# a-slide/Quade

Measured on AMD Instinct MI355X. Metric: read-pairs/sec demultiplexed (2x150 bp, dual 8 bp index), higher is better.
Workload: dtype u8

## Files before the change

include/quade_hip.h:

```cpp
#ifndef QUADE_HIP_H
#define QUADE_HIP_H

#include <stdint.h>

#ifdef __cplusplus
extern "C" {
#endif

#define QD_ABI_VERSION 6

#define QD_OK 0
#define QD_ERR_INVALID (-1)
#define QD_ERR_NO_DEVICE (-2)
#define QD_ERR_HIP (-3)
#define QD_ERR_STATE (-4)
#define QD_ERR_UNSUPPORTED (-5)
#define QD_ERR_BARCODE (-6)
#define QD_ERR_FORMAT (-7)

#define QD_CODE_UNDETERMINED 0xFFFFu
#define QD_MAX_WINDOW 64
#define QD_MAX_KEY 32
#define QD_MAX_SAMPLES 32767

// ... 327 lines not shown
int qd_dev_filter(qd_ctx* ctx, const uint8_t* text1, int64_t len1, const uint32_t* recs1, const uint8_t* text2, int64_t len2,
                  const uint32_t* recs2, int64_t n_pairs, const uint16_t* codes, uint8_t* reasons);
int qd_dev_cstats(qd_ctx* ctx, const uint8_t* text1, int64_t len1, const uint32_t* recs1, const uint8_t* text2, int64_t len2,
                  const uint32_t* recs2, int64_t n_pairs, const uint16_t* codes, const uint8_t* drop);
#define QD_DEV_GUARD_BYTE 0xEE
int qd_dev_pack_rows(int device_id, const qd_layout* layout, const uint8_t* const text[2], const int64_t text_len[2],
                     const uint32_t* const recs[2], int64_t n, int64_t short_cap, uint8_t* const seq_rows[2], uint8_t* const qual_rows[2],
                     uint8_t* const len_rows[2], uint32_t* short_idx, int64_t short_room, uint32_t* n_short);
int qd_dev_route_format(int device_id, const qd_plan* plan, int32_t n_samples, int32_t write_pass, int32_t write_fail, int32_t write_undet,
                        const uint8_t* const text[4], const int64_t text_len[4], const uint32_t* const recs[4], const uint16_t* codes,
                        const uint8_t* drop, int64_t n, int32_t shift, uint16_t* dest, uint32_t* len1, uint32_t* len2, uint32_t* perm,
                        uint16_t* sdest, uint32_t* g1, uint32_t* g2, uint32_t* first, uint32_t* g1_first, uint32_t* g2_first, int64_t* base1,
                        int64_t* base2, uint8_t* out, int64_t out_cap, int64_t* out_used);
int qd_dev_pack_members(int device_id, const uint8_t* slots, int64_t stride, const uint32_t* len, int64_t n, uint64_t* offsets, uint8_t* packed,
                        int64_t packed_cap);
int qd_get_plan(const qd_ctx* ctx, qd_plan* out);
int qd_context_device(const qd_ctx* ctx, int32_t* device_id);

#ifdef __cplusplus
}
#endif
#endif
```

quade_amd/csrc/quade_text.hip:

```cpp
#include <hip/hip_runtime.h>

#include "quade_text.h"
#include "text_rules.h"

namespace {

constexpr uint32_t TILE = QD_TEXT_TILE;
constexpr uint32_t LINE_BLOCK = 256;
static_assert(LINE_BLOCK * 64 == TILE, "a lane owns 64 bytes of its tile");

struct __attribute__((packed, aligned(1))) U4 {
    uint32_t x, y, z, w;
};

__device__ __forceinline__ uint32_t nl_bits4(uint32_t w) {
    const uint32_t x = w ^ 0x0A0A0A0Au;
    const uint32_t t = ~(((x & 0x7F7F7F7Fu) + 0x7F7F7F7Fu) | x | 0x7F7F7F7Fu);
    return (((t >> 7) * 0x00204081u) >> 21) & 0xFu;
}

__device__ __forceinline__ uint64_t nl_mask64(const uint8_t* text, uint32_t b, uint32_t len, bool virt) {
    if (b > len) return 0;
    uint64_t m = 0;
    if (b < len) {
        const uint4* p = reinterpret_cast<const uint4*>(text + b);
#pragma unroll
        for (int q = 0; q < 4; ++q) {
            const uint4 v = p[q];
            const uint64_t bits = (uint64_t)nl_bits4(v.x) | ((uint64_t)nl_bits4(v.y) << 4) | ((uint64_t)nl_bits4(v.z) << 8) |
                                  ((uint64_t)nl_bits4(v.w) << 12);
            m |= bits << (16 * q);
        }
        if (len - b < 64) m &= (1ull << (len - b)) - 1;
    }
    if (virt && len - b < 64) m |= 1ull << (len - b);
    return m;
}

__device__ __forceinline__ bool virtual_newline(const uint8_t* text, uint32_t len, int at_eof) {
    return at_eof && len > 0 && text[len - 1] != '\n';
}

__device__ __forceinline__ uint32_t wave_scan_incl(uint32_t v, uint32_t lane) {
#pragma unroll
    for (int d = 1; d < 64; d <<= 1) {
        const uint32_t y = __shfl_up(v, d, 64);
        if (lane >= (uint32_t)d) v += y;
// ... 12 lines not shown
    const uint32_t inc = wave_scan_incl(v, lane);
    if (lane == 63) lds[wave] = inc;
    __syncthreads();
    uint32_t before = 0, all = 0;
#pragma unroll
    for (int i = 0; i < NW; ++i) {
        const uint32_t s = lds[i];
        if ((uint32_t)i < wave) before += s;
        all += s;
    }
    __syncthreads();
    *total = all;
    return before + inc - v;
}

__global__ __launch_bounds__(LINE_BLOCK) void line_count(const uint8_t* text, uint32_t len, int at_eof, uint32_t* tile_counts) {
    __shared__ uint32_t part[LINE_BLOCK / 64];
    const bool virt = virtual_newline(text, len, at_eof);
    const uint32_t b = blockIdx.x * TILE + threadIdx.x * 64u;
    const uint32_t c = wave_sum((uint32_t)__popcll(nl_mask64(text, b, len, virt)));
    if ((threadIdx.x & 63u) == 0) part[threadIdx.x >> 6] = c;
    __syncthreads();
    if (threadIdx.x == 0) tile_counts[blockIdx.x] = part[0] + part[1] + part[2] + part[3];
}

__global__ __launch_bounds__(1024) void scan_single(const uint32_t* in, uint32_t n, uint32_t* out) {
    __shared__ uint32_t lds[16];
    __shared__ uint32_t carry;
    if (threadIdx.x == 0) carry = 0;
    __syncthreads();
    for (uint32_t base = 0; base < n; base += 1024) {
        const uint32_t i = base + threadIdx.x;
        const uint32_t v = i < n ? in[i] : 0u;
        uint32_t total;
        const uint32_t ex = block_scan_excl<16>(v, lds, &total);
        const uint32_t c = carry;
        if (i < n) out[i] = c + ex;
        __syncthreads();
        if (threadIdx.x == 0) carry = c + total;
        __syncthreads();
    }
    if (threadIdx.x == 0) out[n] = carry;
}

struct ScanMany {
    const uint32_t* in[4];
    uint32_t* out[4];
    uint32_t n[4];
};
__global__ __launch_bounds__(1024) void scan_single_many(const ScanMany a) {
    __shared__ uint32_t lds[16];
    __shared__ uint32_t carry;
    const uint32_t* in = a.in[blockIdx.x];
    uint32_t* out = a.out[blockIdx.x];
    const uint32_t n = a.n[blockIdx.x];
    if (threadIdx.x == 0) carry = 0;
    __syncthreads();
    for (uint32_t base = 0; base < n; base += 1024) {
        const uint32_t i = base + threadIdx.x;
        const uint32_t v = i < n ? in[i] : 0u;
        uint32_t total;
        const uint32_t ex = block_scan_excl<16>(v, lds, &total);
        const uint32_t c = carry;
        if (i < n) out[i] = c + ex;
        __syncthreads();
        if (threadIdx.x == 0) carry = c + total;
        __syncthreads();
    }
    if (threadIdx.x == 0) out[n] = carry;
}
struct DoneMany {
    const uint32_t* a[4];
    const uint32_t* lines[4];
    uint32_t n[4];
    uint32_t cap[4];
    qd_scan_result* r[4];
};
__global__ void lines_done_many(const DoneMany d) {
    const uint32_t w = threadIdx.x;
    const uint32_t n = d.a[w][d.n[w]];
    qd_scan_result* r = d.r[w];
    r->n_lines = n;
    r->n_records = n / 4;
    r->overflow = n > d.cap[w] ? 1u : 0u;
    r->n_short = 0;
}
__global__ void recs_done_many(const DoneMany d) {
    const uint32_t w = threadIdx.x;
    qd_scan_result* r = d.r[w];
    const uint32_t n_rec = r->overflow ? 0u : r->n_records;
    const uint32_t n_tiles = (n_rec + 1024u - 1) / 1024u;
    r->n_kept = n_tiles <= d.n[w] ? d.a[w][n_tiles] : 0u;
    r->tail_start = n_rec ? d.lines[w][4 * n_rec - 1] + 1 : 0u;
}

__global__ void lines_done(const uint32_t* tile_base, uint32_t n_tiles, uint32_t line_cap, qd_scan_result* r) {
    const uint32_t n = tile_base[n_tiles];
    r->n_lines = n;
    r->n_records = n / 4;
    r->overflow = n > line_cap ? 1u : 0u;
    r->n_short = 0;
}

__global__ __launch_bounds__(LINE_BLOCK) void line_write(const uint8_t* text, uint32_t len, int at_eof, const uint32_t* tile_base,
                                                         uint32_t* lines, uint32_t line_cap) {
    __shared__ uint32_t lds[LINE_BLOCK / 64];
    const bool virt = virtual_newline(text, len, at_eof);
    const uint32_t b = blockIdx.x * TILE + threadIdx.x * 64u;
    uint64_t m = nl_mask64(text, b, len, virt);
    uint32_t total;
    uint32_t at = tile_base[blockIdx.x] + block_scan_excl<LINE_BLOCK / 64>((uint32_t)__popcll(m), lds, &total);
    while (m) {
        if (at < line_cap) lines[at] = b + (uint32_t)__builtin_ctzll(m);
        ++at;
        m &= m - 1;
    }
}

constexpr uint32_t REC_TILE = 1024;

struct Lines4 {
    uint32_t head, e0, e1, e2, e3;
};
__device__ __forceinline__ Lines4 record_lines(const uint32_t* lines, uint32_t r) {
    const uint4 e = reinterpret_cast<const uint4*>(lines)[r];
    Lines4 l;
    l.head = r ? lines[4 * r - 1] + 1 : 0u;
    l.e0 = e.x;
    l.e1 = e.y;
    l.e2 = e.z;
    l.e3 = e.w;
    return l;
}
__device__ __forceinline__ bool record_kept(const uint8_t* text, const Lines4& l, uint32_t* seq_len) {
    const uint32_t seq = l.e0 + 1, qual = l.e2 + 1;
    const uint32_t seq_end = (l.e1 > seq && text[l.e1 - 1] == '\r') ? l.e1 - 1 : l.e1;
    const uint32_t qual_end = (l.e3 > qual && text[l.e3 - 1] == '\r') ? l.e3 - 1 : l.e3;
    *seq_len = seq_end - seq;
    return seq_end - seq == qual_end - qual;
}

__global__ __launch_bounds__(256) void rec_count(const uint8_t* text, const uint32_t* lines, const qd_scan_result* res, uint32_t need,
                                                 uint32_t* rec_tile, qd_scan_result* out) {
    __shared__ uint32_t part[4], parts[4];
    const uint32_t n_rec = res->overflow ? 0u : res->n_records;
    uint32_t kept = 0, shorts = 0;
#pragma unroll
    for (int i = 0; i < 4; ++i) {
        const uint32_t r = blockIdx.x * REC_TILE + threadIdx.x * 4u + (uint32_t)i;
        if (r < n_rec) {
            uint32_t sl;
            if (record_kept(text, record_lines(lines, r), &sl)) {
                ++kept;
                shorts += sl < need ? 1u : 0u;
            }
        }
    }
    kept = wave_sum(kept);
    shorts = wave_sum(shorts);
    if ((threadIdx.x & 63u) == 0) {
        part[threadIdx.x >> 6] = kept;
        parts[threadIdx.x >> 6] = shorts;
    }
    __syncthreads();
    if (threadIdx.x == 0) {
        rec_tile[blockIdx.x] = part[0] + part[1] + part[2] + part[3];
        const uint32_t s = parts[0] + parts[1] + parts[2] + parts[3];
        if (s) atomicAdd(&out->n_short, s);
    }
}

__global__ void recs_done(const uint32_t* rec_tile, uint32_t n_tiles_max, const uint32_t* lines, qd_scan_result* r) {
    const uint32_t n_rec = r->overflow ? 0u : r->n_records;
    const uint32_t n_tiles = (n_rec + REC_TILE - 1) / REC_TILE;
    r->n_kept = n_tiles <= n_tiles_max ? rec_tile[n_tiles] : 0u;
    r->tail_start = n_rec ? lines[4 * n_rec - 1] + 1 : 0u;
}

__device__ __forceinline__ void name_of_wide(const uint8_t* text, uint32_t head, uint32_t line_end, uint32_t* name_off, uint32_t* name_len) {
    uint32_t h = head + (line_end > head ? 1u : 0u);
    while (h < line_end && qd_is_blank(text[h])) ++h;
    uint32_t e = h;
    while (e < line_end) {
        uint64_t v;
        __builtin_memcpy(&v, text + e, 8);
        uint32_t k = 8;
#pragma unroll
        for (int i = 7; i >= 0; --i)
            if (qd_is_blank((uint8_t)(v >> (8 * i)))) k = (uint32_t)i;
        e += k;
        if (k < 8) break;
    }
    if (e > line_end) e = line_end;
    *name_off = h;
    *name_len = e - h;
}

__global__ __launch_bounds__(256) void rec_write(const uint8_t* text, const uint32_t* lines, const qd_scan_result* res, int want_names,
                                                 const uint32_t* rec_tile, qd_rec* recs) {
    __shared__ uint32_t lds[4];
    const uint32_t n_rec = res->overflow ? 0u : res->n_records;
    Lines4 l[4];
    uint32_t sl[4];
    bool keep[4];
    uint32_t kept = 0;
#pragma unroll
    for (int i = 0; i < 4; ++i) {
        const uint32_t r = blockIdx.x * REC_TILE + threadIdx.x * 4u + (uint32_t)i;
        keep[i] = false;
        if (r < n_rec) {
            l[i] = record_lines(lines, r);
            keep[i] = record_kept(text, l[i], &sl[i]);
        }
        kept += keep[i] ? 1u : 0u;
    }
    uint32_t total;
    uint32_t at = rec_tile[blockIdx.x] + block_scan_excl<4>(kept, lds, &total);
#pragma unroll
    for (int i = 0; i < 4; ++i) {
        if (!keep[i]) continue;
        qd_rec q;
        q.head = l[i].head;
        q.seq = l[i].e0 + 1;
        q.seq_len = sl[i];
        q.qual = l[i].e2 + 1;
        q.name_off = q.head;
        q.name_len = 0;
        if (want_names) name_of_wide(text, l[i].head, l[i].e0, &q.name_off, &q.name_len);
        recs[at++] = q;
    }
}

__global__ void carry_info(const qd_rec* r0, const qd_rec* r1, const qd_rec* r2, const qd_rec* r3, qd_scan_result* s0, qd_scan_result* s1,
                           qd_scan_result* s2, qd_scan_result* s3, int n_streams, uint32_t n0, uint32_t n1, uint32_t n2, uint32_t n3) {
    const qd_rec* recs[4] = {r0, r1, r2, r3};
    qd_scan_result* res[4] = {s0, s1, s2, s3};
    const uint32_t ns[4] = {n0, n1, n2, n3};
    const int k = (int)threadIdx.x;
    if (k < n_streams) res[k]->carry_start = ns[k] < res[k]->n_kept ? recs[k][ns[k]].head : res[k]->tail_start;
}

__global__ void grain_bounds(const uint32_t* lines, const qd_scan_result* res, const uint32_t* grain_start, uint32_t n_grains, qd_grain_index* out) {
    const uint32_t g = blockIdx.x * blockDim.x + threadIdx.x;
    if (g >= n_grains) return;
// ... 432 lines not shown
    const uint32_t i = blockIdx.x;
    const uint32_t L = len[i];
    const uint32_t b0 = blockIdx.y * COPY_PART;
    if (b0 >= L) return;
    const uint32_t b1 = min(b0 + COPY_PART, L);
    const uint8_t* s = slots + (int64_t)i * stride;
    uint8_t* d = packed + offsets[i];
    uint32_t b = b0 + threadIdx.x * 16u;
    for (; b + 16 <= b1; b += 256 * 16) *reinterpret_cast<U4*>(d + b) = *reinterpret_cast<const U4*>(s + b);
    if (b < b1)
        for (uint32_t q = b; q < b1; ++q) d[q] = s[q];
}

}

hipError_t qd_text_scan(const uint8_t* text, uint32_t len, int at_eof, int want_names, uint32_t need, const qd_scan_scratch& s,
                        qd_scan_result* result, hipStream_t st) {
    const uint32_t n_tiles = len / TILE + 1;
    hipLaunchKernelGGL(line_count, dim3(n_tiles), dim3(LINE_BLOCK), 0, st, text, len, at_eof, s.tile_counts);
    hipLaunchKernelGGL(scan_single, dim3(1), dim3(1024), 0, st, s.tile_counts, n_tiles, s.tile_base);
    hipLaunchKernelGGL(lines_done, dim3(1), dim3(1), 0, st, s.tile_base, n_tiles, s.line_cap, result);
    hipLaunchKernelGGL(line_write, dim3(n_tiles), dim3(LINE_BLOCK), 0, st, text, len, at_eof, s.tile_base, s.lines, s.line_cap);
    const uint32_t rec_cap = s.line_cap / 4;
    const uint32_t rec_tiles = (rec_cap + REC_TILE - 1) / REC_TILE;
    if (rec_tiles) {
        hipLaunchKernelGGL(rec_count, dim3(rec_tiles), dim3(256), 0, st, text, s.lines, result, need, s.rec_tile, result);
        hipLaunchKernelGGL(scan_single, dim3(1), dim3(1024), 0, st, s.rec_tile, rec_tiles, s.rec_tile);
        hipLaunchKernelGGL(recs_done, dim3(1), dim3(1), 0, st, s.rec_tile, rec_tiles, s.lines, result);
        hipLaunchKernelGGL(rec_write, dim3(rec_tiles), dim3(256), 0, st, text, s.lines, result, want_names, s.rec_tile, s.recs);
    } else {
        hipLaunchKernelGGL(recs_done, dim3(1), dim3(1), 0, st, s.rec_tile, 0u, s.lines, result);
    }
    return hipGetLastError();
}

hipError_t qd_text_scan_many(int n_windows, const qd_scan_job* jobs, hipStream_t st) {
    if (n_windows < 1 || n_windows > 4) return hipErrorInvalidValue;
    static_assert(REC_TILE == 1024, "recs_done_many");
    ScanMany sm{}, sr{};
    DoneMany dl{}, dr{};
    uint32_t n_tiles[4], rec_tiles[4];
    bool any_rec = false;
    for (int w = 0; w < n_windows; ++w) {
        const qd_scan_job& j = jobs[w];
        n_tiles[w] = j.len / TILE + 1;
        rec_tiles[w] = (j.s.line_cap / 4 + REC_TILE - 1) / REC_TILE;
        any_rec = any_rec || rec_tiles[w];
        sm.in[w] = j.s.tile_counts, sm.out[w] = j.s.tile_base, sm.n[w] = n_tiles[w];
        sr.in[w] = j.s.rec_tile, sr.out[w] = j.s.rec_tile, sr.n[w] = rec_tiles[w];
        dl.a[w] = j.s.tile_base, dl.n[w] = n_tiles[w], dl.cap[w] = j.s.line_cap, dl.r[w] = j.result;
        dr.a[w] = j.s.rec_tile, dr.lines[w] = j.s.lines, dr.n[w] = rec_tiles[w], dr.r[w] = j.result;
    }
    for (int w = 0; w < n_windows; ++w)
        hipLaunchKernelGGL(line_count, dim3(n_tiles[w]), dim3(LINE_BLOCK), 0, st, jobs[w].text, jobs[w].len, jobs[w].at_eof, jobs[w].s.tile_counts);
    hipLaunchKernelGGL(scan_single_many, dim3(n_windows), dim3(1024), 0, st, sm);
    hipLaunchKernelGGL(lines_done_many, dim3(1), dim3(n_windows), 0, st, dl);
    for (int w = 0; w < n_windows; ++w)
        hipLaunchKernelGGL(line_write, dim3(n_tiles[w]), dim3(LINE_BLOCK), 0, st, jobs[w].text, jobs[w].len, jobs[w].at_eof, jobs[w].s.tile_base, jobs[w].s.lines, jobs[w].s.line_cap);
    for (int w = 0; w < n_windows; ++w)
        if (rec_tiles[w])
            hipLaunchKernelGGL(rec_count, dim3(rec_tiles[w]), dim3(256), 0, st, jobs[w].text, jobs[w].s.lines, jobs[w].result, jobs[w].need, jobs[w].s.rec_tile, jobs[w].result);
    if (any_rec) hipLaunchKernelGGL(scan_single_many, dim3(n_windows), dim3(1024), 0, st, sr);
    hipLaunchKernelGGL(recs_done_many, dim3(1), dim3(n_windows), 0, st, dr);
    for (int w = 0; w < n_windows; ++w)
        if (rec_tiles[w])
            hipLaunchKernelGGL(rec_write, dim3(rec_tiles[w]), dim3(256), 0, st, jobs[w].text, jobs[w].s.lines, jobs[w].result, jobs[w].want_names, jobs[w].s.rec_tile, jobs[w].s.recs);
    return hipGetLastError();
}

hipError_t qd_text_grain_index(const uint8_t* text, const uint32_t* lines, uint32_t line_cap, const qd_scan_result* res, const uint32_t* grain_start,
                               uint32_t n_grains, int at_eof, qd_grain_index* out, hipStream_t st) {
    if (!n_grains) return hipSuccess;
    hipLaunchKernelGGL(grain_bounds, dim3((n_grains + 63) / 64), dim3(64), 0, st, lines, res, grain_start, n_grains, out);
    if (line_cap) hipLaunchKernelGGL(grain_index, dim3((line_cap + 255) / 256), dim3(256), 0, st, text, lines, res, grain_start, n_grains, at_eof, out);
    return hipGetLastError();
}

hipError_t qd_text_carry_info(const qd_rec* const recs[4], qd_scan_result* const results[4], int n_streams, const uint32_t n[4], hipStream_t st) {
    hipLaunchKernelGGL(carry_info, dim3(1), dim3(64), 0, st, recs[0], recs[1], recs[2], recs[3], results[0], results[1], results[2], results[3],
                       n_streams, n[0], n[1], n[2], n[3]);
    return hipGetLastError();
}
// ... 102 lines not shown
```

quade_amd/csrc/quade_text_api.cpp:

```cpp
#include <hip/hip_runtime.h>

#include <cstring>
#include <string>
#include <vector>

#include "../../include/quade_hip.h"
#include "quade_text.h"

namespace {
struct Dev {
    void* p = nullptr;
    ~Dev() {
        if (p) (void)hipFree(p);
    }
    hipError_t alloc(size_t n) { return hipMalloc(&p, n ? n : 16); }
    template <class T>
    T* as() { return static_cast<T*>(p); }
};
#define TCHK(call)                            \
    do {                                      \
        if ((call) != hipSuccess) return QD_ERR_HIP; \
    } while (0)
}

// ... 19 lines not shown
    sc.tile_counts = tc.as<uint32_t>();
    sc.tile_base = tb.as<uint32_t>();
    sc.lines = lines.as<uint32_t>();
    sc.line_cap = (uint32_t)line_cap;
    sc.rec_tile = rt.as<uint32_t>();
    sc.recs = recs.as<qd_rec>();
    TCHK(qd_text_scan(d_text.as<uint8_t>(), len, at_eof, want_names, (uint32_t)need, sc, res.as<qd_scan_result>(), nullptr));
    TCHK(hipDeviceSynchronize());
    qd_scan_result r;
    TCHK(hipMemcpy(&r, res.p, sizeof r, hipMemcpyDeviceToHost));
    memcpy(result_out, &r, sizeof r);
    if (r.overflow) return 0;
    const int64_t n = std::min<int64_t>(r.n_kept, recs_cap);
    if (n && recs_out) TCHK(hipMemcpy(recs_out, recs.p, (size_t)n * sizeof(qd_rec), hipMemcpyDeviceToHost));
    return r.n_kept;
}

int qd_dev_crc32(int device_id, const uint8_t* data, int64_t n, int64_t range_bytes, uint32_t* crc_out) {
    if ((!data && n) || n < 0 || range_bytes < 1 || range_bytes > 65536 || !crc_out) return QD_ERR_INVALID;
    TCHK(hipSetDevice(device_id));
    std::vector<qd_crc_range> ranges;
    for (int64_t a = 0; a < n; a += range_bytes) ranges.push_back(qd_crc_range{(uint64_t)a + 3, (uint32_t)std::min<int64_t>(range_bytes, n - a), 0});
    const uint32_t first[2] = {0, (uint32_t)ranges.size()};
    Dev d, dr, dc, df, out;
    TCHK(d.alloc((size_t)n + 16));
    TCHK(dr.alloc(ranges.size() * sizeof(qd_crc_range)));
    TCHK(dc.alloc(ranges.size() * 4));
    TCHK(df.alloc(8));
    TCHK(out.alloc(4));
    if (n) TCHK(hipMemcpy(d.as<uint8_t>() + 3, data, (size_t)n, hipMemcpyHostToDevice));
// ... 239 lines not shown
```

quade_amd/hip_backend.py:

```python
from __future__ import annotations

import ctypes as C
import os

import numpy as np

_HERE = os.path.dirname(os.path.abspath(__file__))
LIB_PATH = os.path.join(_HERE, "lib", "libquade_hip.so")

QD_OK = 0
QD_ERR_INVALID, QD_ERR_NO_DEVICE, QD_ERR_HIP, QD_ERR_STATE = -1, -2, -3, -4
QD_ERR_UNSUPPORTED, QD_ERR_BARCODE, QD_ERR_FORMAT = -5, -6, -7
QD_UNKNOWN_READ_ERROR = -(1 << 40)
CODE_UNDETERMINED = 0xFFFF


class QuadeHipError(RuntimeError):
    def __init__(self, code, text):
        RuntimeError.__init__(self, "libquade_hip error %d: %s" % (code, text))
        self.code = code


class qd_plan(C.Structure):
    _fields_ = [("dual", C.c_int32), ("min_qual", C.c_int32),
# ... 190 lines not shown
    ("qd_dev_crc32", C.c_int, [C.c_int, _P, C.c_int64, C.c_int64, C.POINTER(C.c_uint32)]),
    ("qd_pool_trim", C.c_int, []),
    ("qd_dev_gunzip", C.c_int, [C.c_int, _P, C.c_int64, _P, C.c_int64, C.POINTER(C.c_int64), C.c_int64, C.c_int64, C.c_int64, C.POINTER(C.c_int64)]),
    ("qd_dev_sort_by_dest", C.c_int, [C.c_int, _P, C.c_int64, C.c_int32, _P, _P, _P]),
    ("qd_dev_qstats", C.c_int, [_P, _P, C.c_int64, _P, _P, C.c_int64, _P, C.c_int64, _P]),
    ("qd_dev_clip", C.c_int, [_P, _P, C.c_int64, _P, _P, C.c_int64, _P, C.c_int64, _P, _P]),
    ("qd_dev_trim", C.c_int, [_P, _P, C.c_int64, _P, _P, C.c_int64, _P, C.c_int64, _P, _P]),
    ("qd_dev_pairtrim", C.c_int, [_P, _P, C.c_int64, _P, _P, C.c_int64, _P, C.c_int64, _P, _P]),
    ("qd_dev_filter", C.c_int, [_P, _P, C.c_int64, _P, _P, C.c_int64, _P, C.c_int64, _P, _P]),
    ("qd_dev_cstats", C.c_int, [_P, _P, C.c_int64, _P, _P, C.c_int64, _P, C.c_int64, _P, _P]),
    ("qd_dev_pack_rows", C.c_int, [C.c_int, C.POINTER(qd_layout), _P * 2, C.c_int64 * 2, _P * 2, C.c_int64, C.c_int64, _P * 2, _P * 2, _P * 2,
                                   _P, C.c_int64, C.POINTER(C.c_uint32)]),
    ("qd_dev_route_format", C.c_int, [C.c_int, C.POINTER(qd_plan), C.c_int32, C.c_int32, C.c_int32, C.c_int32, _P * 4, C.c_int64 * 4, _P * 4, _P, _P,
                                      C.c_int64, C.c_int32] + [_P] * 13 + [C.c_int64, C.POINTER(C.c_int64)]),
    ("qd_dev_pack_members", C.c_int, [C.c_int, _P, C.c_int64, _P, C.c_int64, _P, _P, C.c_int64]),
    ("qd_get_plan", C.c_int, [_P, C.POINTER(qd_plan)]),
    ("qd_context_device", C.c_int, [_P, C.POINTER(C.c_int32)]),
]

_lib = None


def load_library(path=None):
    global _lib
    if _lib is not None and path is None:
        return _lib
    default = path is None
    path = path or os.environ.get("QUADE_HIP_LIB") or LIB_PATH
    if not os.path.exists(path):
        raise ImportError(
# ... 854 lines not shown
def dev_pack_members(slots, stride, lens, packed_cap, device_id=0):
    lib = load_library()
    lens = np.ascontiguousarray(lens, dtype=np.uint32)
    slots = np.ascontiguousarray(slots, dtype=np.uint8)
    n = lens.size
    assert slots.size >= n * int(stride)
    offsets = np.zeros(n + 1, dtype=np.uint64)
    packed = np.zeros(max(int(packed_cap), 1), dtype=np.uint8)
    rc = lib.qd_dev_pack_members(int(device_id), _ptr(slots) if n else None, int(stride), _ptr(lens) if n else None, n, _ptr(offsets), _ptr(packed),
                                 int(packed_cap))
    if rc != QD_OK:
        raise QuadeHipError(rc, "qd_dev_pack_members: " + lib.qd_strerror(rc).decode())
    return offsets, packed[:int(packed_cap)]


class Pipe(object):

    def __init__(self, engine, batch_pairs=None):
        self.lib = load_library()
        self.engine = engine
        h = _P()
        r = self.lib.qd_pipe_create(engine._h, C.byref(h))
        if r != QD_OK:
            raise QuadeHipError(r, self.lib.qd_pipe_last_error(None).decode())
        self._h = h
        if batch_pairs:
            self.set_option("batch_pairs", batch_pairs)

    def set_option(self, name, value):
        r = self.lib.qd_pipe_set_option(self._h, name.encode(), int(value))
# ... 58 lines not shown
```

Baseline: 177.4 billion.

## Batch FASTQ scan kernels across windows and skip record compaction when none dropped

The line-count, line-write and record kernels now take all windows in one launch, with each block finding its window from a per-window first-block table. The separate scan and done kernels are merged, which cuts the number of kernel launches. Tiles also record whether they contain any carriage return, so the common CR-free case can skip the per-record CR check. A new fused rec_pass writes records directly and counts drops, so the count, scan and compacting write run only when some record was actually dropped. The cost is extra indirection per block, and a drop-count flag that every later kernel must read before it can exit early.

Measured after the change: 177.2 billion. Within noise of the previous version (-0.1%).

```diff
diff --git a/include/quade_hip.h b/include/quade_hip.h
--- a/include/quade_hip.h
+++ b/include/quade_hip.h
@@ -365,6 +365,10 @@
                         int64_t* base2, uint8_t* out, int64_t out_cap, int64_t* out_used);
 int qd_dev_pack_members(int device_id, const uint8_t* slots, int64_t stride, const uint32_t* len, int64_t n, uint64_t* offsets, uint8_t* packed,
                         int64_t packed_cap);
+int qd_dev_fastq_scan_many(int device_id, int32_t n_windows, const uint8_t* const text[4], const int64_t text_len[4], const int32_t at_eof[4],
+                           const int32_t want_names[4], const int32_t need[4], const int64_t line_cap[4], uint32_t* const lines_out[4],
+                           uint32_t* const recs_out[4], const int64_t recs_cap[4], uint32_t* result_out, int32_t* guards_changed,
+                           int32_t timed_runs, float* ms_out);
 int qd_get_plan(const qd_ctx* ctx, qd_plan* out);
 int qd_context_device(const qd_ctx* ctx, int32_t* device_id);
 
diff --git a/quade_amd/csrc/quade_text.hip b/quade_amd/csrc/quade_text.hip
--- a/quade_amd/csrc/quade_text.hip
+++ b/quade_amd/csrc/quade_text.hip
@@ -1,4 +1,6 @@
 #include <hip/hip_runtime.h>
+
+#include <algorithm>
 
 #include "quade_text.h"
 #include "text_rules.h"
@@ -18,19 +20,27 @@
     const uint32_t t = ~(((x & 0x7F7F7F7Fu) + 0x7F7F7F7Fu) | x | 0x7F7F7F7Fu);
     return (((t >> 7) * 0x00204081u) >> 21) & 0xFu;
 }
-
-__device__ __forceinline__ uint64_t nl_mask64(const uint8_t* text, uint32_t b, uint32_t len, bool virt) {
+__device__ __forceinline__ uint32_t cr_in4(uint32_t w) {
+    const uint32_t x = w ^ 0x0D0D0D0Du;
+    return (x - 0x01010101u) & ~x & 0x80808080u;
+}
+
+__device__ __forceinline__ uint64_t nl_mask64(const uint8_t* text, uint32_t b, uint32_t len, bool virt, uint32_t* cr = nullptr) {
+    if (cr) *cr = 0;
     if (b > len) return 0;
     uint64_t m = 0;
     if (b < len) {
         const uint4* p = reinterpret_cast<const uint4*>(text + b);
+        uint32_t any_cr = 0;
 #pragma unroll
         for (int q = 0; q < 4; ++q) {
             const uint4 v = p[q];
             const uint64_t bits = (uint64_t)nl_bits4(v.x) | ((uint64_t)nl_bits4(v.y) << 4) | ((uint64_t)nl_bits4(v.z) << 8) |
                                   ((uint64_t)nl_bits4(v.w) << 12);
             m |= bits << (16 * q);
-        }
+            any_cr |= cr_in4(v.x) | cr_in4(v.y) | cr_in4(v.z) | cr_in4(v.w);
+        }
+        if (cr) *cr = any_cr;
         if (len - b < 64) m &= (1ull << (len - b)) - 1;
     }
     if (virt && len - b < 64) m |= 1ull << (len - b);
@@ -73,102 +83,105 @@
     return before + inc - v;
 }
 
-__global__ __launch_bounds__(LINE_BLOCK) void line_count(const uint8_t* text, uint32_t len, int at_eof, uint32_t* tile_counts) {
-    __shared__ uint32_t part[LINE_BLOCK / 64];
-    const bool virt = virtual_newline(text, len, at_eof);
-    const uint32_t b = blockIdx.x * TILE + threadIdx.x * 64u;
-    const uint32_t c = wave_sum((uint32_t)__popcll(nl_mask64(text, b, len, virt)));
-    if ((threadIdx.x & 63u) == 0) part[threadIdx.x >> 6] = c;
-    __syncthreads();
-    if (threadIdx.x == 0) tile_counts[blockIdx.x] = part[0] + part[1] + part[2] + part[3];
-}
-
+__device__ __forceinline__ uint32_t scan_words(const uint32_t* in, uint32_t n, uint32_t* out, uint32_t* lds , uint32_t* carry,
+                                               uint32_t mask = 0xFFFFFFFFu, uint32_t* rest = nullptr) {
+    uint32_t others = 0;
+    if (threadIdx.x == 0) *carry = 0;
+    __syncthreads();
+    for (uint32_t base = 0; base < n; base += 1024) {
+        const uint32_t i = base + threadIdx.x;
+        const uint32_t word = i < n ? in[i] : 0u;
+        const uint32_t v = word & mask;
+        others |= word & ~mask;
+        uint32_t total;
+        const uint32_t ex = block_scan_excl<16>(v, lds, &total);
+        const uint32_t c = *carry;
+        if (i < n) out[i] = c + ex;
+        __syncthreads();
+        if (threadIdx.x == 0) *carry = c + total;
+        __syncthreads();
+    }
+    const uint32_t all = *carry;
+    if (threadIdx.x == 0) out[n] = all;
+    if (rest) *rest = others;
+    return all;
+}
 __global__ __launch_bounds__(1024) void scan_single(const uint32_t* in, uint32_t n, uint32_t* out) {
     __shared__ uint32_t lds[16];
     __shared__ uint32_t carry;
-    if (threadIdx.x == 0) carry = 0;
-    __syncthreads();
-    for (uint32_t base = 0; base < n; base += 1024) {
-        const uint32_t i = base + threadIdx.x;
-        const uint32_t v = i < n ? in[i] : 0u;
-        uint32_t total;
-        const uint32_t ex = block_scan_excl<16>(v, lds, &total);
-        const uint32_t c = carry;
-        if (i < n) out[i] = c + ex;
-        __syncthreads();
-        if (threadIdx.x == 0) carry = c + total;
-        __syncthreads();
-    }
-    if (threadIdx.x == 0) out[n] = carry;
-}
-
-struct ScanMany {
-    const uint32_t* in[4];
-    uint32_t* out[4];
-    uint32_t n[4];
+    scan_words(in, n, out, lds, &carry);
+}
+
+__device__ __forceinline__ uint32_t window_of(const uint32_t first[5], uint32_t block) {
+    return (block >= first[1] ? 1u : 0u) + (block >= first[2] ? 1u : 0u) + (block >= first[3] ? 1u : 0u);
+}
+
+struct LineJobs {
+    const uint8_t* text[4];
+    uint32_t len[4];
+    int at_eof[4];
+    uint32_t* tile_counts[4];
+    const uint32_t* tile_base[4];
+    uint32_t* lines[4];
+    uint32_t line_cap[4];
+    uint32_t first[5];
 };
-__global__ __launch_bounds__(1024) void scan_single_many(const ScanMany a) {
+
+constexpr uint32_t TILE_HAS_CR = 0x80000000u;
+__global__ __launch_bounds__(LINE_BLOCK) void line_count(const LineJobs j) {
+    __shared__ uint32_t part[LINE_BLOCK / 64];
+    const uint32_t w = window_of(j.first, blockIdx.x), tile = blockIdx.x - j.first[w];
+    const uint8_t* text = j.text[w];
+    const uint32_t len = j.len[w], lane = threadIdx.x & 63u, wave = threadIdx.x >> 6;
+    const bool virt = virtual_newline(text, len, j.at_eof[w]);
+    uint32_t cr;
+    uint32_t c = wave_sum((uint32_t)__popcll(nl_mask64(text, tile * TILE + threadIdx.x * 64u, len, virt, &cr)));
+    if (__any(cr != 0)) c |= TILE_HAS_CR;
+    if (lane == 0) part[wave] = c;
+    __syncthreads();
+    if (threadIdx.x == 0) {
+        const uint32_t cr_bit = (part[0] | part[1] | part[2] | part[3]) & TILE_HAS_CR;
+        j.tile_counts[w][tile] = (((part[0] & ~TILE_HAS_CR) + (part[1] & ~TILE_HAS_CR) + (part[2] & ~TILE_HAS_CR) + (part[3] & ~TILE_HAS_CR))) | cr_bit;
+    }
+}
+
+struct LineScan {
+    const uint32_t* tile_counts[4];
+    uint32_t* tile_base[4];
+    uint32_t n_tiles[4];
+    uint32_t line_cap[4];
+    uint32_t* dropped[4];
+    qd_scan_result* r[4];
+};
+__global__ __launch_bounds__(1024) void line_scan(const LineScan a) {
     __shared__ uint32_t lds[16];
     __shared__ uint32_t carry;
-    const uint32_t* in = a.in[blockIdx.x];
-    uint32_t* out = a.out[blockIdx.x];
-    const uint32_t n = a.n[blockIdx.x];
-    if (threadIdx.x == 0) carry = 0;
-    __syncthreads();
-    for (uint32_t base = 0; base < n; base += 1024) {
-        const uint32_t i = base + threadIdx.x;
-        const uint32_t v = i < n ? in[i] : 0u;
-        uint32_t total;
-        const uint32_t ex = block_scan_excl<16>(v, lds, &total);
-        const uint32_t c = carry;
-        if (i < n) out[i] = c + ex;
-        __syncthreads();
-        if (threadIdx.x == 0) carry = c + total;
-        __syncthreads();
-    }
-    if (threadIdx.x == 0) out[n] = carry;
-}
-struct DoneMany {
-    const uint32_t* a[4];
-    const uint32_t* lines[4];
-    uint32_t n[4];
-    uint32_t cap[4];
-    qd_scan_result* r[4];
-};
-__global__ void lines_done_many(const DoneMany d) {
-    const uint32_t w = threadIdx.x;
-    const uint32_t n = d.a[w][d.n[w]];
-    qd_scan_result* r = d.r[w];
-    r->n_lines = n;
-    r->n_records = n / 4;
-    r->overflow = n > d.cap[w] ? 1u : 0u;
-    r->n_short = 0;
-}
-__global__ void recs_done_many(const DoneMany d) {
-    const uint32_t w = threadIdx.x;
-    qd_scan_result* r = d.r[w];
-    const uint32_t n_rec = r->overflow ? 0u : r->n_records;
-    const uint32_t n_tiles = (n_rec + 1024u - 1) / 1024u;
-    r->n_kept = n_tiles <= d.n[w] ? d.a[w][n_tiles] : 0u;
-    r->tail_start = n_rec ? d.lines[w][4 * n_rec - 1] + 1 : 0u;
-}
-
-__global__ void lines_done(const uint32_t* tile_base, uint32_t n_tiles, uint32_t line_cap, qd_scan_result* r) {
-    const uint32_t n = tile_base[n_tiles];
-    r->n_lines = n;
-    r->n_records = n / 4;
-    r->overflow = n > line_cap ? 1u : 0u;
-    r->n_short = 0;
-}
-
-__global__ __launch_bounds__(LINE_BLOCK) void line_write(const uint8_t* text, uint32_t len, int at_eof, const uint32_t* tile_base,
-                                                         uint32_t* lines, uint32_t line_cap) {
+    const uint32_t w = blockIdx.x;
+    uint32_t cr;
+    const uint32_t n = scan_words(a.tile_counts[w], a.n_tiles[w], a.tile_base[w], lds, &carry, ~TILE_HAS_CR, &cr);
+    cr = (uint32_t)__syncthreads_or((int)(cr != 0));
+    if (threadIdx.x == 0) {
+        qd_scan_result* r = a.r[w];
+        r->n_lines = n;
+        r->n_records = n / 4;
+        r->overflow = n > a.line_cap[w] ? 1u : 0u;
+        r->n_short = 0;
+        a.dropped[w][0] = 0;
+        a.dropped[w][1] = cr;
+    }
+}
+
+__global__ __launch_bounds__(LINE_BLOCK) void line_write(const LineJobs j) {
     __shared__ uint32_t lds[LINE_BLOCK / 64];
-    const bool virt = virtual_newline(text, len, at_eof);
-    const uint32_t b = blockIdx.x * TILE + threadIdx.x * 64u;
+    const uint32_t w = window_of(j.first, blockIdx.x), tile = blockIdx.x - j.first[w];
+    const uint8_t* text = j.text[w];
+    const uint32_t len = j.len[w], line_cap = j.line_cap[w];
+    uint32_t* lines = j.lines[w];
+    const bool virt = virtual_newline(text, len, j.at_eof[w]);
+    const uint32_t b = tile * TILE + threadIdx.x * 64u;
     uint64_t m = nl_mask64(text, b, len, virt);
     uint32_t total;
-    uint32_t at = tile_base[blockIdx.x] + block_scan_excl<LINE_BLOCK / 64>((uint32_t)__popcll(m), lds, &total);
+    uint32_t at = j.tile_base[w][tile] + block_scan_excl<LINE_BLOCK / 64>((uint32_t)__popcll(m), lds, &total);
     while (m) {
         if (at < line_cap) lines[at] = b + (uint32_t)__builtin_ctzll(m);
         ++at;
@@ -191,49 +204,12 @@
     l.e3 = e.w;
     return l;
 }
-__device__ __forceinline__ bool record_kept(const uint8_t* text, const Lines4& l, uint32_t* seq_len) {
+__device__ __forceinline__ bool record_kept(const uint8_t* text, const Lines4& l, uint32_t* seq_len, bool has_cr = true) {
     const uint32_t seq = l.e0 + 1, qual = l.e2 + 1;
-    const uint32_t seq_end = (l.e1 > seq && text[l.e1 - 1] == '\r') ? l.e1 - 1 : l.e1;
-    const uint32_t qual_end = (l.e3 > qual && text[l.e3 - 1] == '\r') ? l.e3 - 1 : l.e3;
+    const uint32_t seq_end = (has_cr && l.e1 > seq && text[l.e1 - 1] == '\r') ? l.e1 - 1 : l.e1;
+    const uint32_t qual_end = (has_cr && l.e3 > qual && text[l.e3 - 1] == '\r') ? l.e3 - 1 : l.e3;
     *seq_len = seq_end - seq;
     return seq_end - seq == qual_end - qual;
-}
-
-__global__ __launch_bounds__(256) void rec_count(const uint8_t* text, const uint32_t* lines, const qd_scan_result* res, uint32_t need,
-                                                 uint32_t* rec_tile, qd_scan_result* out) {
-    __shared__ uint32_t part[4], parts[4];
-    const uint32_t n_rec = res->overflow ? 0u : res->n_records;
-    uint32_t kept = 0, shorts = 0;
-#pragma unroll
-    for (int i = 0; i < 4; ++i) {
-        const uint32_t r = blockIdx.x * REC_TILE + threadIdx.x * 4u + (uint32_t)i;
-        if (r < n_rec) {
-            uint32_t sl;
-            if (record_kept(text, record_lines(lines, r), &sl)) {
-                ++kept;
-                shorts += sl < need ? 1u : 0u;
-            }
-        }
-    }
-    kept = wave_sum(kept);
-    shorts = wave_sum(shorts);
-    if ((threadIdx.x & 63u) == 0) {
-        part[threadIdx.x >> 6] = kept;
-        parts[threadIdx.x >> 6] = shorts;
-    }
-    __syncthreads();
-    if (threadIdx.x == 0) {
-        rec_tile[blockIdx.x] = part[0] + part[1] + part[2] + part[3];
-        const uint32_t s = parts[0] + parts[1] + parts[2] + parts[3];
-        if (s) atomicAdd(&out->n_short, s);
-    }
-}
-
-__global__ void recs_done(const uint32_t* rec_tile, uint32_t n_tiles_max, const uint32_t* lines, qd_scan_result* r) {
-    const uint32_t n_rec = r->overflow ? 0u : r->n_records;
-    const uint32_t n_tiles = (n_rec + REC_TILE - 1) / REC_TILE;
-    r->n_kept = n_tiles <= n_tiles_max ? rec_tile[n_tiles] : 0u;
-    r->tail_start = n_rec ? lines[4 * n_rec - 1] + 1 : 0u;
 }
 
 __device__ __forceinline__ void name_of_wide(const uint8_t* text, uint32_t head, uint32_t line_end, uint32_t* name_off, uint32_t* name_len) {
@@ -254,18 +230,132 @@
     *name_off = h;
     *name_len = e - h;
 }
-
-__global__ __launch_bounds__(256) void rec_write(const uint8_t* text, const uint32_t* lines, const qd_scan_result* res, int want_names,
-                                                 const uint32_t* rec_tile, qd_rec* recs) {
+__device__ __forceinline__ qd_rec record_of(const uint8_t* text, const Lines4& l, uint32_t seq_len, int want_names) {
+    qd_rec q;
+    q.head = l.head;
+    q.seq = l.e0 + 1;
+    q.seq_len = seq_len;
+    q.qual = l.e2 + 1;
+    q.name_off = q.head;
+    q.name_len = 0;
+    if (want_names) name_of_wide(text, l.head, l.e0, &q.name_off, &q.name_len);
+    return q;
+}
+
+struct RecJobs {
+    const uint8_t* text[4];
+    const uint32_t* lines[4];
+    qd_scan_result* res[4];
+    uint32_t need[4];
+    int want_names[4];
+    uint32_t* rec_tile[4];
+    qd_rec* recs[4];
+    uint32_t* dropped[4];
+    uint32_t first[5];
+};
+
+__global__ __launch_bounds__(256) void rec_pass(const RecJobs j) {
+    __shared__ uint32_t part[4], parts[4];
+    const uint32_t w = window_of(j.first, blockIdx.x), tile = blockIdx.x - j.first[w];
+    qd_scan_result* res = j.res[w];
+    const uint32_t n_rec = res->overflow ? 0u : res->n_records;
+    if (tile * REC_TILE >= n_rec) return;
+    const uint8_t* text = j.text[w];
+    const uint32_t* lines = j.lines[w];
+    const uint32_t need = j.need[w];
+    const int want_names = j.want_names[w];
+    qd_rec* recs = j.recs[w];
+    const bool has_cr = j.dropped[w][1] != 0;
+    uint32_t drops = 0, shorts = 0;
+#pragma unroll
+    for (uint32_t i = 0; i < 4; ++i) {
+        const uint32_t r = tile * REC_TILE + i * 256u + threadIdx.x;
+        if (r >= n_rec) continue;
+        const Lines4 l = record_lines(lines, r);
+        uint32_t sl;
+        if (record_kept(text, l, &sl, has_cr)) {
+            shorts += sl < need ? 1u : 0u;
+            recs[r] = record_of(text, l, sl, want_names);
+        } else {
+            ++drops;
+        }
+    }
+    drops = wave_sum(drops);
+    shorts = wave_sum(shorts);
+    if ((threadIdx.x & 63u) == 0) {
+        part[threadIdx.x >> 6] = drops;
+        parts[threadIdx.x >> 6] = shorts;
+    }
+    __syncthreads();
+    if (threadIdx.x == 0) {
+        const uint32_t d = part[0] + part[1] + part[2] + part[3], s = parts[0] + parts[1] + parts[2] + parts[3];
+        if (d) atomicAdd(j.dropped[w], d);
+        if (s) atomicAdd(&res->n_short, s);
+    }
+}
+
+__global__ __launch_bounds__(256) void rec_count(const RecJobs j) {
+    __shared__ uint32_t part[4];
+    const uint32_t w = window_of(j.first, blockIdx.x), tile = blockIdx.x - j.first[w];
+    if (*j.dropped[w] == 0) return;
+    const qd_scan_result* res = j.res[w];
+    const uint32_t n_rec = res->overflow ? 0u : res->n_records;
+    if (tile * REC_TILE >= n_rec) return;
+    const uint8_t* text = j.text[w];
+    const uint32_t* lines = j.lines[w];
+    uint32_t kept = 0;
+#pragma unroll
+    for (int i = 0; i < 4; ++i) {
+        const uint32_t r = tile * REC_TILE + threadIdx.x * 4u + (uint32_t)i;
+        if (r < n_rec) {
+            uint32_t sl;
+            kept += record_kept(text, record_lines(lines, r), &sl) ? 1u : 0u;
+        }
+    }
+    kept = wave_sum(kept);
+    if ((threadIdx.x & 63u) == 0) part[threadIdx.x >> 6] = kept;
+    __syncthreads();
+    if (threadIdx.x == 0) j.rec_tile[w][tile] = part[0] + part[1] + part[2] + part[3];
+}
+
+struct RecScan {
+    uint32_t* rec_tile[4];
+    const uint32_t* lines[4];
+    const uint32_t* dropped[4];
+    qd_scan_result* r[4];
+};
+__global__ __launch_bounds__(1024) void rec_scan(const RecScan a) {
+    __shared__ uint32_t lds[16];
+    __shared__ uint32_t carry;
+    const uint32_t w = blockIdx.x;
+    qd_scan_result* r = a.r[w];
+    const uint32_t n_rec = r->overflow ? 0u : r->n_records;
+    uint32_t n_kept = n_rec;
+    if (*a.dropped[w] != 0) n_kept = scan_words(a.rec_tile[w], (n_rec + REC_TILE - 1) / REC_TILE, a.rec_tile[w], lds, &carry);
+    if (threadIdx.x == 0) {
+        r->n_kept = n_kept;
+        r->tail_start = n_rec ? a.lines[w][4 * n_rec - 1] + 1 : 0u;
+    }
+}
+
+__global__ __launch_bounds__(256) void rec_write(const RecJobs j) {
     __shared__ uint32_t lds[4];
+    const uint32_t w = window_of(j.first, blockIdx.x), tile = blockIdx.x - j.first[w];
+    if (*j.dropped[w] == 0) return;
+    const qd_scan_result* res = j.res[w];
     const uint32_t n_rec = res->overflow ? 0u : res->n_records;
+    if (tile * REC_TILE >= n_rec) return;
+    const uint8_t* text = j.text[w];
+    const uint32_t* lines = j.lines[w];
+    const int want_names = j.want_names[w];
+    qd_rec* recs = j.recs[w];
     Lines4 l[4];
     uint32_t sl[4];
     bool keep[4];
     uint32_t kept = 0;
 #pragma unroll
     for (int i = 0; i < 4; ++i) {
-        const uint32_t r = blockIdx.x * REC_TILE + threadIdx.x * 4u + (uint32_t)i;
+        const uint32_t r = tile * REC_TILE + threadIdx.x * 4u + (uint32_t)i;
         keep[i] = false;
         if (r < n_rec) {
             l[i] = record_lines(lines, r);
@@ -274,19 +364,11 @@
         kept += keep[i] ? 1u : 0u;
     }
     uint32_t total;
-    uint32_t at = rec_tile[blockIdx.x] + block_scan_excl<4>(kept, lds, &total);
+    uint32_t at = j.rec_tile[w][tile] + block_scan_excl<4>(kept, lds, &total);
 #pragma unroll
     for (int i = 0; i < 4; ++i) {
         if (!keep[i]) continue;
-        qd_rec q;
-        q.head = l[i].head;
-        q.seq = l[i].e0 + 1;
-        q.seq_len = sl[i];
-        q.qual = l[i].e2 + 1;
-        q.name_off = q.head;
-        q.name_len = 0;
-        if (want_names) name_of_wide(text, l[i].head, l[i].e0, &q.name_off, &q.name_len);
-        recs[at++] = q;
+        recs[at++] = record_of(text, l[i], sl[i], want_names);
     }
 }
 
@@ -749,58 +831,45 @@
 
 }
 
+hipError_t qd_text_scan_many(int n_windows, const qd_scan_job* jobs, hipStream_t st) {
+    if (n_windows < 1 || n_windows > 4) return hipErrorInvalidValue;
+    LineJobs lj{};
+    LineScan ls{};
+    RecJobs rj{};
+    RecScan rs{};
+    uint32_t line_tiles = 0, rec_tiles = 0;
+    for (int w = 0; w < n_windows; ++w) {
+        const qd_scan_job& j = jobs[w];
+        const uint32_t n_tiles = j.len / TILE + 1;
+        const uint32_t rec_cap = (uint32_t)std::min<uint64_t>(j.s.line_cap, (uint64_t)j.len + 1) / 4;
+        uint32_t* dropped = j.s.tile_counts + n_tiles;
+        lj.text[w] = j.text, lj.len[w] = j.len, lj.at_eof[w] = j.at_eof, lj.tile_counts[w] = j.s.tile_counts, lj.tile_base[w] = j.s.tile_base;
+        lj.lines[w] = j.s.lines, lj.line_cap[w] = j.s.line_cap, lj.first[w] = line_tiles;
+        ls.tile_counts[w] = j.s.tile_counts, ls.tile_base[w] = j.s.tile_base, ls.n_tiles[w] = n_tiles, ls.line_cap[w] = j.s.line_cap;
+        ls.dropped[w] = dropped, ls.r[w] = j.result;
+        rj.text[w] = j.text, rj.lines[w] = j.s.lines, rj.res[w] = j.result, rj.need[w] = j.need, rj.want_names[w] = j.want_names;
+        rj.rec_tile[w] = j.s.rec_tile, rj.recs[w] = j.s.recs, rj.dropped[w] = dropped, rj.first[w] = rec_tiles;
+        rs.rec_tile[w] = j.s.rec_tile, rs.lines[w] = j.s.lines, rs.dropped[w] = dropped, rs.r[w] = j.result;
+        line_tiles += n_tiles;
+        rec_tiles += (rec_cap + REC_TILE - 1) / REC_TILE;
+    }
+    for (int w = n_windows; w < 5; ++w) lj.first[w] = line_tiles, rj.first[w] = rec_tiles;
+    hipLaunchKernelGGL(line_count, dim3(line_tiles), dim3(LINE_BLOCK), 0, st, lj);
+    hipLaunchKernelGGL(line_scan, dim3(n_windows), dim3(1024), 0, st, ls);
+    hipLaunchKernelGGL(line_write, dim3(line_tiles), dim3(LINE_BLOCK), 0, st, lj);
+    if (rec_tiles) {
+        hipLaunchKernelGGL(rec_pass, dim3(rec_tiles), dim3(256), 0, st, rj);
+        hipLaunchKernelGGL(rec_count, dim3(rec_tiles), dim3(256), 0, st, rj);
+    }
+    hipLaunchKernelGGL(rec_scan, dim3(n_windows), dim3(1024), 0, st, rs);
+    if (rec_tiles) hipLaunchKernelGGL(rec_write, dim3(rec_tiles), dim3(256), 0, st, rj);
+    return hipGetLastError();
+}
+
 hipError_t qd_text_scan(const uint8_t* text, uint32_t len, int at_eof, int want_names, uint32_t need, const qd_scan_scratch& s,
                         qd_scan_result* result, hipStream_t st) {
-    const uint32_t n_tiles = len / TILE + 1;
-    hipLaunchKernelGGL(line_count, dim3(n_tiles), dim3(LINE_BLOCK), 0, st, text, len, at_eof, s.tile_counts);
-    hipLaunchKernelGGL(scan_single, dim3(1), dim3(1024), 0, st, s.tile_counts, n_tiles, s.tile_base);
-    hipLaunchKernelGGL(lines_done, dim3(1), dim3(1), 0, st, s.tile_base, n_tiles, s.line_cap, result);
-    hipLaunchKernelGGL(line_write, dim3(n_tiles), dim3(LINE_BLOCK), 0, st, text, len, at_eof, s.tile_base, s.lines, s.line_cap);
-    const uint32_t rec_cap = s.line_cap / 4;
-    const uint32_t rec_tiles = (rec_cap + REC_TILE - 1) / REC_TILE;
-    if (rec_tiles) {
-        hipLaunchKernelGGL(rec_count, dim3(rec_tiles), dim3(256), 0, st, text, s.lines, result, need, s.rec_tile, result);
-        hipLaunchKernelGGL(scan_single, dim3(1), dim3(1024), 0, st, s.rec_tile, rec_tiles, s.rec_tile);
-        hipLaunchKernelGGL(recs_done, dim3(1), dim3(1), 0, st, s.rec_tile, rec_tiles, s.lines, result);
-        hipLaunchKernelGGL(rec_write, dim3(rec_tiles), dim3(256), 0, st, text, s.lines, result, want_names, s.rec_tile, s.recs);
-    } else {
-        hipLaunchKernelGGL(recs_done, dim3(1), dim3(1), 0, st, s.rec_tile, 0u, s.lines, result);
-    }
-    return hipGetLastError();
-}
-
-hipError_t qd_text_scan_many(int n_windows, const qd_scan_job* jobs, hipStream_t st) {
-    if (n_windows < 1 || n_windows > 4) return hipErrorInvalidValue;
-    static_assert(REC_TILE == 1024, "recs_done_many");
-    ScanMany sm{}, sr{};
-    DoneMany dl{}, dr{};
-    uint32_t n_tiles[4], rec_tiles[4];
-    bool any_rec = false;
-    for (int w = 0; w < n_windows; ++w) {
-        const qd_scan_job& j = jobs[w];
-        n_tiles[w] = j.len / TILE + 1;
-        rec_tiles[w] = (j.s.line_cap / 4 + REC_TILE - 1) / REC_TILE;
-        any_rec = any_rec || rec_tiles[w];
-        sm.in[w] = j.s.tile_counts, sm.out[w] = j.s.tile_base, sm.n[w] = n_tiles[w];
-        sr.in[w] = j.s.rec_tile, sr.out[w] = j.s.rec_tile, sr.n[w] = rec_tiles[w];
-        dl.a[w] = j.s.tile_base, dl.n[w] = n_tiles[w], dl.cap[w] = j.s.line_cap, dl.r[w] = j.result;
-        dr.a[w] = j.s.rec_tile, dr.lines[w] = j.s.lines, dr.n[w] = rec_tiles[w], dr.r[w] = j.result;
-    }
-    for (int w = 0; w < n_windows; ++w)
-        hipLaunchKernelGGL(line_count, dim3(n_tiles[w]), dim3(LINE_BLOCK), 0, st, jobs[w].text, jobs[w].len, jobs[w].at_eof, jobs[w].s.tile_counts);
-    hipLaunchKernelGGL(scan_single_many, dim3(n_windows), dim3(1024), 0, st, sm);
-    hipLaunchKernelGGL(lines_done_many, dim3(1), dim3(n_windows), 0, st, dl);
-    for (int w = 0; w < n_windows; ++w)
-        hipLaunchKernelGGL(line_write, dim3(n_tiles[w]), dim3(LINE_BLOCK), 0, st, jobs[w].text, jobs[w].len, jobs[w].at_eof, jobs[w].s.tile_base, jobs[w].s.lines, jobs[w].s.line_cap);
-    for (int w = 0; w < n_windows; ++w)
-        if (rec_tiles[w])
-            hipLaunchKernelGGL(rec_count, dim3(rec_tiles[w]), dim3(256), 0, st, jobs[w].text, jobs[w].s.lines, jobs[w].result, jobs[w].need, jobs[w].s.rec_tile, jobs[w].result);
-    if (any_rec) hipLaunchKernelGGL(scan_single_many, dim3(n_windows), dim3(1024), 0, st, sr);
-    hipLaunchKernelGGL(recs_done_many, dim3(1), dim3(n_windows), 0, st, dr);
-    for (int w = 0; w < n_windows; ++w)
-        if (rec_tiles[w])
-            hipLaunchKernelGGL(rec_write, dim3(rec_tiles[w]), dim3(256), 0, st, jobs[w].text, jobs[w].s.lines, jobs[w].result, jobs[w].want_names, jobs[w].s.rec_tile, jobs[w].s.recs);
-    return hipGetLastError();
+    const qd_scan_job job{text, len, at_eof, want_names, need, s, result};
+    return qd_text_scan_many(1, &job, st);
 }
 
 hipError_t qd_text_grain_index(const uint8_t* text, const uint32_t* lines, uint32_t line_cap, const qd_scan_result* res, const uint32_t* grain_start,
diff --git a/quade_amd/csrc/quade_text_api.cpp b/quade_amd/csrc/quade_text_api.cpp
--- a/quade_amd/csrc/quade_text_api.cpp
+++ b/quade_amd/csrc/quade_text_api.cpp
@@ -1,5 +1,6 @@
 #include <hip/hip_runtime.h>
 
+#include <algorithm>
 #include <cstring>
 #include <string>
 #include <vector>
@@ -57,6 +58,86 @@
     const int64_t n = std::min<int64_t>(r.n_kept, recs_cap);
     if (n && recs_out) TCHK(hipMemcpy(recs_out, recs.p, (size_t)n * sizeof(qd_rec), hipMemcpyDeviceToHost));
     return r.n_kept;
+}
+
+int qd_dev_fastq_scan_many(int device_id, int32_t n_windows, const uint8_t* const text[4], const int64_t text_len[4], const int32_t at_eof[4],
+                           const int32_t want_names[4], const int32_t need[4], const int64_t line_cap[4], uint32_t* const lines_out[4],
+                           uint32_t* const recs_out[4], const int64_t recs_cap[4], uint32_t* result_out, int32_t* guards_changed,
+                           int32_t timed_runs, float* ms_out) {
+    constexpr size_t GUARD = 64;
+    if (n_windows < 1 || n_windows > 4 || !text || !text_len || !at_eof || !want_names || !need || !line_cap || !result_out) return QD_ERR_INVALID;
+    if (timed_runs < 0 || timed_runs > 1000 || (timed_runs && !ms_out)) return QD_ERR_INVALID;
+    for (int w = 0; w < n_windows; ++w)
+        if (text_len[w] < 0 || text_len[w] > (int64_t)1 << 30 || (!text[w] && text_len[w]) || line_cap[w] < 4 || line_cap[w] > (int64_t)1 << 30 ||
+            (recs_out && recs_out[w] && (!recs_cap || recs_cap[w] < 0)))
+            return QD_ERR_INVALID;
+    TCHK(hipSetDevice(device_id));
+    Dev d_text[4], tc[4], tb[4], lines[4], rt[4], recs[4], res;
+    qd_scan_job jobs[4];
+    size_t cap[4];
+    TCHK(res.alloc(4 * sizeof(qd_scan_result)));
+    TCHK(hipMemset(res.p, 0xFF, 4 * sizeof(qd_scan_result)));
+    for (int w = 0; w < n_windows; ++w) {
+        const uint32_t len = (uint32_t)text_len[w], n_tiles = len / QD_TEXT_TILE + 1;
+        cap[w] = (size_t)(line_cap[w] & ~(int64_t)3);
+        TCHK(d_text[w].alloc((size_t)len + 2 * QD_TEXT_TILE));
+        TCHK(tc[w].alloc((size_t)(n_tiles + 2) * 4));
+        TCHK(tb[w].alloc((size_t)(n_tiles + 2) * 4));
+        TCHK(lines[w].alloc((cap[w] + GUARD) * 4));
+        TCHK(rt[w].alloc((cap[w] / 4 / 1024 + 4) * 4));
+        TCHK(recs[w].alloc((cap[w] / 4 + GUARD) * sizeof(qd_rec)));
+        TCHK(hipMemset(d_text[w].p, '\n', (size_t)len + 2 * QD_TEXT_TILE));
+        TCHK(hipMemset(lines[w].p, QD_DEV_GUARD_BYTE, (cap[w] + GUARD) * 4));
+        TCHK(hipMemset(recs[w].p, QD_DEV_GUARD_BYTE, (cap[w] / 4 + GUARD) * sizeof(qd_rec)));
+        if (len) TCHK(hipMemcpy(d_text[w].p, text[w], len, hipMemcpyHostToDevice));
+        qd_scan_scratch sc;
+        sc.tile_counts = tc[w].as<uint32_t>();
+        sc.tile_base = tb[w].as<uint32_t>();
+        sc.lines = lines[w].as<uint32_t>();
+        sc.line_cap = (uint32_t)cap[w];
+        sc.rec_tile = rt[w].as<uint32_t>();
+        sc.recs = recs[w].as<qd_rec>();
+        jobs[w] = qd_scan_job{d_text[w].as<uint8_t>(), len, at_eof[w], want_names[w], (uint32_t)need[w], sc, res.as<qd_scan_result>() + w};
+    }
+    TCHK(qd_text_scan_many(n_windows, jobs, nullptr));
+    TCHK(hipDeviceSynchronize());
+    if (timed_runs) {
+        hipEvent_t e0, e1;
+        TCHK(hipEventCreate(&e0));
+        TCHK(hipEventCreate(&e1));
+        hipError_t err = hipSuccess;
+        for (int k = -2; k < timed_runs && err == hipSuccess; ++k) {
+            err = hipEventRecord(e0, nullptr);
+            if (err == hipSuccess) err = qd_text_scan_many(n_windows, jobs, nullptr);
+            if (err == hipSuccess) err = hipEventRecord(e1, nullptr);
+            if (err == hipSuccess) err = hipEventSynchronize(e1);
+            float ms = 0;
+            if (err == hipSuccess) err = hipEventElapsedTime(&ms, e0, e1);
+            if (k >= 0) ms_out[k] = ms;
+        }
+        (void)hipEventDestroy(e0);
+        (void)hipEventDestroy(e1);
+        TCHK(err);
+    }
+    std::vector<uint8_t> guard;
+    for (int w = 0; w < n_windows; ++w) {
+        qd_scan_result r;
+        TCHK(hipMemcpy(&r, res.as<qd_scan_result>() + w, sizeof r, hipMemcpyDeviceToHost));
+        memcpy(result_out + 8 * w, &r, sizeof r);
+        int32_t changed = 0;
+        guard.resize(GUARD * sizeof(qd_rec));
+        TCHK(hipMemcpy(guard.data(), lines[w].as<uint32_t>() + cap[w], GUARD * 4, hipMemcpyDeviceToHost));
+        for (size_t i = 0; i < GUARD * 4; ++i) changed += guard[i] != QD_DEV_GUARD_BYTE;
+        TCHK(hipMemcpy(guard.data(), recs[w].as<qd_rec>() + cap[w] / 4, GUARD * sizeof(qd_rec), hipMemcpyDeviceToHost));
+        for (size_t i = 0; i < GUARD * sizeof(qd_rec); ++i) changed += guard[i] != QD_DEV_GUARD_BYTE;
+        if (guards_changed) guards_changed[w] = changed;
+        if (lines_out && lines_out[w]) TCHK(hipMemcpy(lines_out[w], lines[w].p, cap[w] * 4, hipMemcpyDeviceToHost));
+        if (recs_out && recs_out[w]) {
+            const size_t n = std::min<size_t>(cap[w] / 4, (size_t)recs_cap[w]);
+            if (n) TCHK(hipMemcpy(recs_out[w], recs[w].p, n * sizeof(qd_rec), hipMemcpyDeviceToHost));
+        }
+    }
+    return QD_OK;
 }
 
 int qd_dev_crc32(int device_id, const uint8_t* data, int64_t n, int64_t range_bytes, uint32_t* crc_out) {
diff --git a/quade_amd/hip_backend.py b/quade_amd/hip_backend.py
--- a/quade_amd/hip_backend.py
+++ b/quade_amd/hip_backend.py
@@ -228,6 +228,7 @@
     ("qd_dev_route_format", C.c_int, [C.c_int, C.POINTER(qd_plan), C.c_int32, C.c_int32, C.c_int32, C.c_int32, _P * 4, C.c_int64 * 4, _P * 4, _P, _P,
                                       C.c_int64, C.c_int32] + [_P] * 13 + [C.c_int64, C.POINTER(C.c_int64)]),
     ("qd_dev_pack_members", C.c_int, [C.c_int, _P, C.c_int64, _P, C.c_int64, _P, _P, C.c_int64]),
+    ("qd_dev_fastq_scan_many", C.c_int, [C.c_int, C.c_int32, _P, _P, _P, _P, _P, _P, _P, _P, _P, _P, _P, C.c_int32, _P]),
     ("qd_get_plan", C.c_int, [_P, C.POINTER(qd_plan)]),
     ("qd_context_device", C.c_int, [_P, C.POINTER(C.c_int32)]),
 ]
@@ -1112,6 +1113,33 @@
     return offsets, packed[:int(packed_cap)]
 
 
+def dev_fastq_scan_many(texts, at_eof, want_names, need, line_cap, timed_runs=0, device_id=0):
+    lib = load_library()
+    n = len(texts)
+    assert 1 <= n <= 4 and len(at_eof) == len(want_names) == len(need) == len(line_cap) == n
+    bufs = [np.frombuffer(t, dtype=np.uint8) if len(t) else np.zeros(1, np.uint8) for t in texts]
+    caps = [int(c) & ~3 for c in line_cap]
+    lines = [np.zeros(max(c, 4), dtype=np.uint32) for c in caps]
+    recs = [np.zeros((max(c // 4, 1), 6), dtype=np.uint32) for c in caps]
+
+    def ptrs(arrays):
+        return (C.c_void_p * 4)(*([_ptr(a) for a in arrays] + [None] * (4 - n)))
+
+    def ints(ctype, values):
+        return (ctype * 4)(*([int(v) for v in values] + [0] * (4 - n)))
+
+    result = np.zeros((n, 8), dtype=np.uint32)
+    guards = np.zeros(4, dtype=np.int32)
+    ms = np.zeros(max(int(timed_runs), 1), dtype=np.float32)
+    rc = lib.qd_dev_fastq_scan_many(int(device_id), n, ptrs(bufs), ints(C.c_int64, [len(t) for t in texts]), ints(C.c_int32, at_eof),
+                                    ints(C.c_int32, want_names), ints(C.c_int32, need), ints(C.c_int64, line_cap), ptrs(lines), ptrs(recs),
+                                    ints(C.c_int64, [c // 4 for c in caps]), _ptr(result), _ptr(guards), int(timed_runs), _ptr(ms))
+    if rc != QD_OK:
+        raise QuadeHipError(rc, "qd_dev_fastq_scan_many: " + lib.qd_strerror(rc).decode())
+    out = [{"lines": lines[w][:caps[w]], "recs": recs[w][:caps[w] // 4], "result": result[w], "guards_changed": int(guards[w])} for w in range(n)]
+    return (out, [float(x) for x in ms[:int(timed_runs)]]) if timed_runs else out
+
+
 class Pipe(object):
 
     def __init__(self, engine, batch_pairs=None):
```
